# fenghansen/YOND_public

Hardware: AMD Instinct MI355X
Metric: Bayer megapixels/sec end-to-end (NLE+VST+denoise+iVST) (higher is better)
Workload: dtype f32 (3x3 convolutions: f32 operands as two f16 halves -- 22-23 significant bits -- on the f16 MFMA, 3 products per f32 product, f32 accumulate; per-layer error vs float64 asserted <= 2x the f32 direct kernel's and <= 2e-5 of max|ref| (tests/test_hip_conv.py; measured 1.3e-6 vs 1.5e-6), whole frame v

## Files before the change

### include/yond_hip.h

```cpp
#ifndef YOND_HIP_H
#define YOND_HIP_H

#include <stddef.h>
#include <stdint.h>

#ifdef __cplusplus
extern "C" {
#endif

#define YOND_OK 0
#define YOND_EINVAL (-1)
#define YOND_EUNSUPPORTED (-2)

#define YOND_ABI_VERSION 8
int yond_abi_version(void);

int yond_pack_vst_norm_f32(const float* bayer, int H, int W, float* out, int pad_l, int pad_r, int pad_t,
                           int pad_b, int mode, double scale, double gain, double sigma, double lo,
                           double hi, const double* lut_x, const float* lut_y, int lut_n, float* img_max,
                           void* stream);

int yond_pack_vst_norm_biaslut_f32(const float* bayer, int H, int W, float* out, int pad_l, int pad_r, int pad_t,
                                   int pad_b, double scale, double gain, double sigma, double lo, double hi,
                                   const double* lut_x, const double* lut_y, int lut_n, float* img_max, void* stream);
// ... 48 lines not shown
    int kc;
    int algo;
    const float* out4_w;
    const float* out4_b;
    const float* out4_x;
    const float* out4_ub;
    float* out4_dst;
    unsigned int* status;
    int in_fmt, out_fmt;
    int res_fmt;
    unsigned long long* clk;
    int tile_order;
    float* dst2;
} YondConvDesc;
#define YOND_STATUS_HALF_OVERFLOW 1u
#define YOND_FMT_NHWC_F32 0
#define YOND_FMT_SPLIT_PLANES 1
#define YOND_FMT_PLANES4 2
#define YOND_SP_PLANE_UNITS(H, W) ((((H) * (W)) + 8) / 8 * 8)
#define YOND_SP_BYTES(N, C, H, W) ((size_t)(N) * ((C) / 16) * 4 * (size_t)YOND_SP_PLANE_UNITS(H, W) * 16)
#define YOND_HP_BYTES(N, C, H, W) ((size_t)(N) * ((C) / 16) * 2 * (size_t)YOND_SP_PLANE_UNITS(H, W) * 16)

int yond_conv_config(int ksize, int stride, int cin, int cout, int shuffle, int N, int Ho, int Wo, int* tn, int* kc);
int yond_pack_conv_weight_f32(const float* w, int cout, int cin, int ksize, int tn, int kc, float* dst);
int yond_pack_conv_weight_split_f32(const float* w, int cout, int cin, int ksize, int tn, int kc, float* dst);
int yond_conv2d_f32(const YondConvDesc* desc, void* stream);

int yond_conv_wino_supported(int cin, int cout);
int yond_pack_conv_wino_weight_f32(const float* w, int cout, int cin, int tn, float* dst);

int yond_conv_split_supported(int ksize, int stride, int cin, int cout);
int yond_pack_conv_split_weight_f32(const float* w, int cout, int cin, int ksize, int tn, int parts, float* dst);
int yond_gemm_k1_stationary_supported(const YondConvDesc* desc);
int yond_pack_conv_split_weight_dev_f32(const float* w, int cout, int cin, int ksize, int tn, int parts, float* dst, int* status,
                                        void* stream);
int yond_pack_conv_split_weights_batch_dev_f32(const float* src, const long long* desc, int nlayers, float* dst, size_t ngroups,
                                               int* status, void* stream);

int yond_conv_in_f32(const float* x, const float* ub , int N, int H, int W, int Cout,
                     const float* wpk, const float* bias, float slope, float* dst,
                     int out_fmt , void* stream);
int yond_pack_conv_in_weight_f32(const float* w , int cout, float* dst );

int yond_conv_out_f32(const float* feat , int Cin, const float* w ,
                      const float* bias , const float* x ,
                      const float* ub , int N, int H, int W, float* dst ,
                      void* stream);

int yond_maxpool2_f32(const float* src, int N, int H, int W, int C, float* dst, void* stream);

typedef struct YondFilmDesc {
    int kind, C, ld;
    const float *w_a0, *b_a0, *w_a2, *b_a2;
    const float *w_b0, *b_b0;
    const float *w_b, *b_b;
    const float *cb1, *cb2;
    float *s1, *t1, *s2, *t2;
} YondFilmDesc;
int yond_film_f32(const YondFilmDesc* descs, int nblocks, const float* t , const float* ub ,
                  int N, void* stream);

int yond_box_stats_self1_f32(const float* bayer, int H, int W, int k, int k2, int tile_w, float* mean,
                             float* var, float* blur2, void* stream);
int yond_box_stats_self2_f32(const float* blur2, int h, int w, int k, int tile_w, float* lap, void* stream);
int yond_box_stats_collab_f32(const float* bayer_lr, const float* bayer_hr, int H, int W, int k, int tile_w,
                              float* mean, float* var, float* lap, void* stream);
// ... 234 lines not shown
```

### yond_public_amd/_lib.py

```python
import ctypes as C
import os

import torch

_HERE = os.path.dirname(os.path.abspath(__file__))
LIB_PATH = os.environ.get("YOND_HIP_LIB", os.path.join(_HERE, "libyond_hip.so"))
_lib = None
ABI_VERSION = 8

vp, i32, f32, f64, sz, i64 = C.c_void_p, C.c_int, C.c_float, C.c_double, C.c_size_t, C.c_longlong


class YondConvDesc(C.Structure):
    _fields_ = [("src0", vp), ("src1", vp), ("C0", i32), ("C1", i32), ("N", i32), ("H", i32), ("W", i32),
                ("Ho", i32), ("Wo", i32), ("Cout", i32), ("ksize", i32), ("stride", i32), ("shuffle", i32),
                ("pre_act", i32), ("post_act", i32), ("slope", f32), ("wpk", vp), ("escale", vp),
                ("eshift", vp), ("ebatch", i32), ("res", vp), ("dst", vp), ("tn", i32), ("kc", i32), ("algo", i32),
                ("out4_w", vp), ("out4_b", vp), ("out4_x", vp), ("out4_ub", vp), ("out4_dst", vp), ("status", vp),
                ("in_fmt", i32), ("out_fmt", i32), ("res_fmt", i32), ("clk", vp), ("tile_order", i32), ("dst2", vp)]


class YondBlock0Desc(C.Structure):
    _fields_ = [("x", vp), ("in_fmt", i32), ("N", i32), ("H", i32), ("W", i32), ("w1", vp), ("w2", vp),
                ("s1", vp), ("t1", vp), ("s2", vp), ("t2", vp), ("ebatch", i32), ("dst", vp),
# ... 2 lines not shown

class YondFilmDesc(C.Structure):
    _fields_ = [("kind", i32), ("C", i32), ("ld", i32),
                ("w_a0", vp), ("b_a0", vp), ("w_a2", vp), ("b_a2", vp), ("w_b0", vp), ("b_b0", vp),
                ("w_b", vp), ("b_b", vp), ("cb1", vp), ("cb2", vp),
                ("s1", vp), ("t1", vp), ("s2", vp), ("t2", vp)]


PROTOTYPES = {
    "yond_abi_version": [],
    "yond_pack_vst_norm_f32": [vp, i32, i32, vp, i32, i32, i32, i32, i32, f64, f64, f64, f64, f64, vp, vp, i32, vp, vp],
    "yond_pack_vst_norm_biaslut_f32": [vp, i32, i32, vp, i32, i32, i32, i32, f64, f64, f64, f64, f64, vp, vp, i32, vp, vp],
    "yond_bias_eval_f32": [vp, sz, vp, vp, i32, i32, i32, f64, f64, vp, vp],
    "yond_denorm_ivst_unpack_f32": [vp, i32, i32, i32, i32, i32, i32, vp, i32, f64, f64, f64, f64, f64, i32, vp],
    "yond_pack_vst_norm_batch_f32": [vp, i32, i32, i32, vp, i32, i32, i32, i32, f64, f64, f64, f64, f64, vp, vp, i32, i32, vp, vp],
    "yond_denorm_ivst_unpack_batch_f32": [vp, i32, i32, i32, i32, i32, i32, i32, vp, i32, f64, f64, f64, f64, f64, i32, vp],
    "yond_vst_elem_f32": [vp, sz, f64, f64, f64, vp, vp],
    "yond_ivst_elem_f64": [vp, sz, f64, f64, i32, vp, vp],
    "yond_bayer2rggb_f32": [vp, i32, i32, vp, vp],
    "yond_rggb2bayer_f32": [vp, i32, i32, vp, vp],
    "yond_rot90_f32": [vp, i32, i32, i32, i32, vp, vp],
    "yond_nchw4_to_nhwc4_f32": [vp, vp, i32, i32, i32, vp],
    "yond_nhwc4_to_nchw4_f32": [vp, vp, i32, i32, i32, vp],
    "yond_image_max_f32": [vp, i32, sz, vp, vp, vp],
    "yond_conv_config": [i32, i32, i32, i32, i32, i32, i32, i32, C.POINTER(i32), C.POINTER(i32)],
    "yond_pack_conv_weight_f32": [vp, i32, i32, i32, i32, i32, vp],
    "yond_conv2d_f32": [C.POINTER(YondConvDesc), vp],
    "yond_conv_wino_supported": [i32, i32],
    "yond_pack_conv_wino_weight_f32": [vp, i32, i32, i32, vp],
    "yond_pack_conv_weight_split_f32": [vp, i32, i32, i32, i32, i32, vp],
    "yond_conv_split_supported": [i32, i32, i32, i32],
    "yond_pack_conv_split_weight_f32": [vp, i32, i32, i32, i32, i32, vp],
    "yond_gemm_k1_stationary_supported": [C.POINTER(YondConvDesc)],
    "yond_pack_conv_split_weight_dev_f32": [vp, i32, i32, i32, i32, i32, vp, vp, vp],
    "yond_pack_conv_split_weights_batch_dev_f32": [vp, vp, i32, vp, sz, vp, vp],
    "yond_conv_in_f32": [vp, vp, i32, i32, i32, i32, vp, vp, f32, vp, i32, vp],
    "yond_pack_conv_in_weight_f32": [vp, i32, vp],
    "yond_conv_out_f32": [vp, i32, vp, vp, vp, vp, i32, i32, i32, vp, vp],
    "yond_maxpool2_f32": [vp, i32, i32, i32, i32, vp, vp],
    "yond_film_f32": [vp, i32, vp, vp, i32, vp],
    "yond_box_stats_self1_f32": [vp, i32, i32, i32, i32, i32, vp, vp, vp, vp],
    "yond_box_stats_self2_f32": [vp, i32, i32, i32, i32, vp, vp],
    "yond_box_stats_collab_f32": [vp, vp, i32, i32, i32, i32, vp, vp, vp, vp],
    "yond_box_stats_self_stats_f32": [vp, i32, i32, i32, i32, i32, vp, vp, vp, vp, vp, i32, vp, vp],
    "yond_box_stats_collab_stats_f32": [vp, vp, i32, i32, i32, i32, vp, vp, vp, vp, i32, vp, vp],
    "yond_select_ws_bytes": [i32],
    "yond_select_ranks_f32": [vp, sz, vp, i32, vp, vp, vp],
    "yond_percentiles_f32": [vp, sz, vp, i32, vp, vp, vp],
    "yond_nle_ws_bytes": [sz],
    "yond_nle_stats_f32": [vp, vp, sz, i32, vp, i32, vp, vp],
    "yond_nle_threshold_f32": [vp, sz, vp, i32, i32, vp, vp],
    "yond_nle_state_layout": [vp],
    "yond_nle_moments_f32": [vp, vp, vp, sz, vp, vp],
    "yond_nlf_occupancy_f32": [vp, vp, sz, i32, vp, i32, vp, vp],
    "yond_nlf_score3_f64": [vp, vp, vp, i32, vp, vp, vp],
    "yond_nlf_moments_f32": [vp, vp, vp, sz, vp, vp, vp],
    "yond_bias_lut_f64": [vp, i32, f64, f64, vp, vp],
    "yond_block_metrics_tiles": [i32, i32],
    "yond_block_metrics_f32": [vp, vp, i32, i32, i32, i32, vp, vp],
    "yond_block_metrics_rgb8": [vp, vp, i32, i32, i32, i32, vp, vp],
    "yond_render_srgb": [vp, i32, i32, i32, i32, i32, C.POINTER(f64), C.POINTER(f64), i32, vp, vp, i32, vp, f64, vp],
    "yond_clock_probe": [f64, vp, vp],
    "yond_img2raw_f32": [vp, sz, i32, i32, i32, vp, vp, i32, i32, i32, vp, vp, vp, vp],
    "yond_pg_noise_f32": [vp, vp, sz, i32, vp, i32, vp],
    "yond_camera_noise_f32": [vp, vp, sz, i32, vp, i32, i32, vp],
    "yond_est_conv_in_f32": [vp, i32, i32, i32, i32, vp, vp, vp, vp],
# ... 133 lines not shown
```

### yond_public_amd/csrc/conv.hip

```cpp
#include "common.h"
#include <cstdlib>

#ifndef YOND_B32_WGS
#define YOND_B32_WGS 2
#endif
#ifndef YOND_ABL
#define YOND_ABL 0
#endif

template <int KS, int STRIDE, int TH, int TN, int KC>
struct ConvCfg {
    static constexpr int TW = 32;
    static constexpr int TAPS = KS * KS;
    static constexpr int PADK = KS / 2;
    static constexpr int IH = (TH - 1) * STRIDE + KS;
    static constexpr int IW = (TW - 1) * STRIDE + KS;
    static constexpr int HALF = (IW + 1) / 2;
    static constexpr int TWP = (STRIDE == 2) ? 2 * HALF : IW;
    static constexpr int PS = KC + 4;
    static constexpr int IN_FLOATS = IH * TWP * PS;
    static constexpr int Q = KC / 8;
    static constexpr int W_FLOATS = TAPS * Q * 2 * TN * 4;
    static constexpr int BUF_FLOATS = IN_FLOATS + W_FLOATS;
    static constexpr int NW = TN / 32;
// ... 487 lines not shown
            for (int tap = 0; tap < taps; ++tap)
                for (int q = 0; q < Q; ++q)
                    for (int h = 0; h < 2; ++h)
                        for (int j = 0; j < tn; ++j)
                            for (int e = 0; e < 4; ++e) {
                                const int co = ct * tn + j, ci = ch * kc + q * 8 + h * 4 + e;
                                dst[o++] = w[((size_t)co * cin + ci) * taps + tap];
                            }
    return YOND_OK;
}

extern "C" int yond_pack_conv_weight_split_f32(const float* w, int cout, int cin, int ksize, int tn, int kc, float* dst) {
    const int rc = yond_pack_conv_weight_f32(w, cout, cin, ksize, tn, kc, dst);
    if (rc != YOND_OK) return rc;
    const size_t n = (size_t)cout * cin * ksize * ksize;
    for (size_t i = 0; i < n; ++i)
        if (!(fabsf(w[i]) <= 65504.0f)) return YOND_EUNSUPPORTED;
    for (size_t i = 0; i < n; ++i) {
        const float v = dst[i];
        const _Float16 h = (_Float16)v;
        const _Float16 l = (_Float16)((v - (float)h) * 2048.0f);
        unsigned short hb, lb;
        __builtin_memcpy(&hb, &h, 2);
        __builtin_memcpy(&lb, &l, 2);
        const unsigned u = (unsigned)hb | ((unsigned)lb << 16);
        __builtin_memcpy(&dst[i], &u, 4);
    }
    return YOND_OK;
}

int yond_conv_wino_dispatch(const YondConvDesc& d, hipStream_t st);
int yond_conv_split_dispatch(const YondConvDesc& d, hipStream_t st);
int yond_gemm_k1_stationary_dispatch(const YondConvDesc& d, hipStream_t st);

extern "C" int yond_conv2d_f32(const YondConvDesc* dp, void* stream) {
    if (!dp) return YOND_EINVAL;
    const YondConvDesc& d = *dp;
    hipStream_t st = (hipStream_t)stream;
    if (!d.src0 || !(d.dst || d.out4_dst) || !d.wpk || d.N <= 0 || d.H <= 0 || d.W <= 0 || d.Ho <= 0 || d.Wo <= 0) return YOND_EINVAL;
    if (d.out4_dst && ((d.algo != 3 && d.algo != 4) || !d.out4_w || d.Cout != 32 || d.stride != 1)) return YOND_EUNSUPPORTED;
    if (d.C1 > 0 && !d.src1) return YOND_EINVAL;
    if (d.shuffle < 0 || d.shuffle > 2) return YOND_EINVAL;
    if (d.shuffle == 2 && d.algo != 3 && d.algo != 4 && d.algo != 6) return YOND_EUNSUPPORTED;
    if ((long long)d.N * d.H * d.W > 0x7fffffffLL) return YOND_EUNSUPPORTED;
    if (d.pre_act != 0 && d.pre_act != 1) return YOND_EINVAL;
    if (d.in_fmt < 0 || d.in_fmt > 2 || d.out_fmt < 0 || d.out_fmt > 2 || (d.res_fmt != 0 && d.res_fmt != 2)) return YOND_EINVAL;
    if (d.algo == 6) return yond_gemm_k1_stationary_dispatch(d, st);
    if ((d.in_fmt || d.out_fmt || d.res_fmt) && d.algo != 3 && d.algo != 4) return YOND_EUNSUPPORTED;
    if (d.algo == 1) return yond_conv_wino_dispatch(d, st);
    if (d.algo == 3 || d.algo == 4) return yond_conv_split_dispatch(d, st);
    if (d.algo != 0 && d.algo != 2 && d.algo != 5) return YOND_EINVAL;
    if (d.tn != 32 && d.tn != 64) return YOND_EINVAL;
    int tn, kc;
    const int rc = yond_conv_config(d.ksize, d.stride, d.C0 + d.C1, d.Cout, d.shuffle, 0, 0, 0, &tn, &kc);
    if (rc != YOND_OK) return rc;
    tn = d.tn;
    if (d.kc != 0) kc = d.kc;
    if (kc != 8 && kc != 16) return YOND_EINVAL;
    if (kc == 8 && d.ksize != 3) return YOND_EINVAL;
    if (d.ksize == 3 && d.stride == 2 && kc != 8) return YOND_EINVAL;
    if (d.C0 % kc != 0 || d.C1 % kc != 0 || d.Cout % tn != 0) return YOND_EUNSUPPORTED;
    if (d.shuffle && (d.ksize != 1 || (d.Cout / 4) % tn != 0)) return YOND_EUNSUPPORTED;
    if ((long long)d.N * d.H * d.W > 0x7fffffffLL) return YOND_EUNSUPPORTED;
    if (d.stride == 2) {
        if (d.Ho != (d.H + 1) / 2 || d.Wo != (d.W + 1) / 2) return YOND_EINVAL;
    } else if (d.Ho != d.H || d.Wo != d.W) return YOND_EINVAL;
    if (d.pre_act != 0 && d.pre_act != 1) return YOND_EINVAL;
    if (d.post_act != 0 && d.post_act != 2) return YOND_EUNSUPPORTED;
    if (d.pre_act == 1 && !(d.ksize == 3 && d.stride == 1)) return YOND_EUNSUPPORTED;
    if (d.ksize == 3 && d.stride == 1 && kc == 8) {
        if (d.pre_act) return tn == 64 ? launch_conv<3, 1, 8, 64, 8, true>(d, st) : launch_conv<3, 1, 8, 32, 8, true>(d, st);
        return tn == 64 ? launch_conv<3, 1, 8, 64, 8, false>(d, st) : launch_conv<3, 1, 8, 32, 8, false>(d, st);
    }
    if (d.ksize == 3 && d.stride == 1) {
        if (d.pre_act) return tn == 64 ? launch_conv<3, 1, 8, 64, 16, true>(d, st) : launch_conv<3, 1, 8, 32, 16, true>(d, st);
        return tn == 64 ? launch_conv<3, 1, 8, 64, 16, false>(d, st) : launch_conv<3, 1, 8, 32, 16, false>(d, st);
    }
    if (d.ksize == 3 && d.stride == 2)
        return tn == 64 ? launch_conv<3, 2, 8, 64, 8, false>(d, st) : launch_conv<3, 2, 4, 32, 8, false>(d, st);
    return tn == 64 ? launch_conv<1, 1, 8, 64, 16, false>(d, st) : launch_conv<1, 1, 8, 32, 16, false>(d, st);
// ... 2 lines not shown
```

### yond_public_amd/engine.py

```python
import ctypes as C
import os

import numpy as np
import torch

from . import _lib as L


def _rup(c, m=32):
    return (c + m - 1) // m * m


def _np_ptr(a):
    return C.c_void_p(a.ctypes.data)


FILM_MAX_C = 1024


WINO_DEFAULT = 'split'


SPLIT_PLANES = True
SP_FLOW = True
HALF_FLOW = True
HALF_K1_TN128 = True
HALF_S2_TN128 = True
HALF_FLOW_TN128 = True
HALF_TN128 = True
FUSE_OUT4 = True
FUSE_BLOCK0 = False
K1_SUB2 = True
K1_D2_LEVELS = (3,)
K1_STATIONARY_LEVELS = (2, 1, 0)
K1_D2_LEVELS_HALF = ()
SP_CONV1_MIN_LEVEL = 3
UNET_SP = True
SNAKE_ORDER = True


def sp_plane_units(H, W):
    return (H * W + 8) // 8 * 8


class _PackedConv:

    def __init__(self, dev, weight, bias, ksize, stride, splits, shuffle=False):
        lib = L.load()
        w = weight.detach().to('cpu', torch.float32).numpy()
        if shuffle:
            cin, cout = w.shape[0], w.shape[1]
            coutp = _rup(cout)
            m = np.zeros((4, coutp, cin), np.float32)
            m[:, :cout, :] = w.transpose(2, 3, 1, 0).reshape(4, cout, cin)
            w = m.reshape(4 * coutp, cin, 1, 1)
            self.cout_real_p = coutp
            gemm_n = 4 * coutp
        else:
            cout = w.shape[0]
            coutp = _rup(cout)
            gemm_n = coutp
            self.cout_real_p = coutp
        assert sum(splits) == w.shape[1], (splits, w.shape)
        psplits = [_rup(s) for s in splits]
        cinp = sum(psplits)
        wp = np.zeros((gemm_n, cinp, ksize, ksize), np.float32)
        so, do = 0, 0
# ... 214 lines not shown
            return False
        prec = getattr(self, 'precision', 'fp32')
        if prec not in ('fp32', 'fp16'):
            return False
        parts = 2 if prec == 'fp32' else 1
        return all(pc.ksize == 3 and pc.stride == 1 and pc.split(parts) is not None for pc in (pc1, pc2))

    def _sp_flow(self, N, H, W):
        if not (SPLIT_PLANES and SP_FLOW) or getattr(self, 'strict', False) or getattr(self, 'conv_algo', WINO_DEFAULT) != 'split':
            return False
        prec = getattr(self, 'precision', 'fp32')
        if prec not in ('fp32', 'fp16') or (prec == 'fp16' and not HALF_FLOW) or sp_plane_units(H, W) * 64 * 4 >= 2 ** 31:
            return False
        parts = 2 if prec == 'fp32' else 1
        for i, blk in self.blocks.items():
            for k in ('conv1', 'conv2', 'pool', 'upsc'):
                if k in blk and blk[k].split(parts, wide=False) is None:
                    return False
        return self._out4_fusable(self.blocks[9]['conv2'], flow=True)

    def _out4_fusable(self, pc, flow=False):
        prec = getattr(self, 'precision', 'fp32')
        return (not getattr(self, 'strict', False) and getattr(self, 'conv_algo', WINO_DEFAULT) == 'split' and (prec == 'fp32' or (prec == 'fp16' and flow))
                and pc.ksize == 3 and pc.stride == 1 and pc.gemm_n == 32 and pc.split(2 if prec == 'fp32' else 1) is not None and FUSE_OUT4)

    def _new_sp(self, key, N, H, W, Cc, parts=2):
        cache = self.__dict__.setdefault('_sp_cache', {})
        k = (key, N, H, W, Cc, parts, getattr(self, 'lane', 0))
        if k not in cache:
            cache[k] = torch.zeros(N * (Cc // 16) * 2 * parts * sp_plane_units(H, W) * 4, dtype=torch.float32, device=self.dev)
        return cache[k]

    def _conv(self, pc, src0, src1, N, H, W, dst, escale=None, eshift=None, ebatch=0, res=None, pre_act=0, post_act=0,
              slope=0.0, algo=None, out4=None, in_fmt=0, out_fmt=0, res_fmt=0, dst2=None, stationary=False):
        d = L.YondConvDesc()
        d.src0 = src0.data_ptr()
        d.src1 = src1.data_ptr() if src1 is not None else None
        d.C0 = pc.psplits[0]
        d.C1 = pc.psplits[1] if len(pc.psplits) > 1 else 0
        d.N, d.H, d.W = N, H, W
        if pc.stride == 2:
            d.Ho, d.Wo = (H + 1) // 2, (W + 1) // 2
        else:
            d.Ho, d.Wo = H, W
        d.Cout = pc.gemm_n
        d.ksize, d.stride, d.shuffle = pc.ksize, pc.stride, int(pc.shuffle)
        d.pre_act, d.post_act, d.slope = pre_act, post_act, slope
        prec = getattr(self, 'precision', 'fp32')
        if getattr(self, 'strict', False) and algo is None:
            prec, algo = 'fp32-mfma', 1
        if algo is None:
            algo = getattr(self, 'conv_algo', WINO_DEFAULT)
            if prec == 'fp32-mfma' and algo == 'split':
                algo = 1
            if prec == 'fp16' and WINO_DEFAULT == 'split':
                algo = 'half'
        fp16 = prec == 'fp16' or algo == 'fp16'
        wino = split = None
        if algo in ('split', 'half'):
            ws2 = (HALF_S2_TN128 and algo == 'half' and pc.stride == 2 and in_fmt == 1 and out_fmt == 2 and dst2 is None
                   and (pc.gemm_n // 128) * ((d.Wo + 31) // 32) * ((d.Ho + 7) // 8) * N >= 256)
            ws2 = ws2 or (HALF_K1_TN128 and algo == 'half' and pc.ksize == 1 and in_fmt == 1 and dst2 is None)
            split = pc.split(2 if algo == 'split' else 1, wide=(not (in_fmt or out_fmt or res_fmt or dst2 is not None)) or (HALF_FLOW_TN128 and out_fmt == 1),
                             wide_s2=ws2)
            if algo == 'half' and pc.ksize == 1 and in_fmt != 1:
                split = None
            if split is None and not fp16 and pc.ksize == 3:
                wino = pc.wino()
        elif not fp16:
            wino = pc.wino() if algo in (1, 2) else None
        if split is not None:
            tn, wpk = split
            kc = 16
            d.algo = 3 if algo == 'split' else 4
        elif wino is not None:
            tn, wpk = wino
            kc = 8
            d.algo = 1
        elif algo == 'split' and pc.ksize == 1 and not fp16 and pc.config(N, d.Ho, d.Wo, split=True)[2] is not None:
            tn, kc, wpk = pc.config(N, d.Ho, d.Wo, split=True)
            d.algo = 5
        else:
            tn, kc, wpk = pc.config(N, d.Ho, d.Wo)
            d.algo = 2 if (fp16 and pc.wmax <= 65504.0) else 0
        d.wpk = wpk.data_ptr()
        d.tn = tn
        d.kc = kc
        d.escale = escale.data_ptr() if escale is not None else None
        d.eshift = (eshift if eshift is not None else pc.bias).data_ptr()
        d.ebatch = ebatch
        d.res = res.data_ptr() if res is not None else None
        d.dst = dst.data_ptr() if dst is not None else None
        status = getattr(self, 'status', None)
        d.status = status.data_ptr() + 4 * self.status_slot if status is not None else None
        d.in_fmt, d.out_fmt, d.res_fmt = in_fmt, out_fmt, res_fmt
        d.dst2 = dst2.data_ptr() if dst2 is not None else None
        if stationary and d.algo == 3 and self.lib.yond_gemm_k1_stationary_supported(C.byref(d)):
            d.algo = 6
        if SNAKE_ORDER and d.algo in (3, 4, 6):
            self._tile_order = 1 - getattr(self, '_tile_order', 0)
            d.tile_order = self._tile_order
        clk = getattr(self, 'clk', None)
        d.clk = clk.data_ptr() if (clk is not None and d.algo in (3, 4, 6)) else None
        if (in_fmt or out_fmt or res_fmt) and d.algo not in (3, 4, 6):
            raise L.YondHipError("split-plane / 4-channel-plane tensors need the split-operand kernel (algo 3, or 4 with h-only planes)")
        if out4 is not None:
            w4, b4, x4, ub4, o4 = out4
            if d.algo not in (3, 4):
                raise L.YondHipError("fused output projection needs the split-operand 3x3 kernel")
            d.out4_w, d.out4_b = w4.data_ptr(), (b4.data_ptr() if b4 is not None else None)
            d.out4_x = x4.data_ptr() if x4 is not None else None
            d.out4_ub = ub4.data_ptr() if ub4 is not None else None
            d.out4_dst = o4.data_ptr()
        prof = getattr(self, 'prof', None)
        if prof is not None:
            tag = f"conv_wino_kernel<{tn}>" if d.algo == 1 else f"conv_mfma_kernel<{pc.ksize},{pc.stride},8,{tn},{kc}>"
            if d.algo in (3, 4, 6):
                tag = f"conv_split_kernel<{pc.stride if pc.ksize == 3 else 'k1'},{tn},{1 if d.algo == 4 else 2}>" + ("/stationary" if d.algo == 6 else "")
            if d.algo == 2:
                tag += "/f16"
            if d.algo == 5:
                tag += "/split"
            only = getattr(self, 'prof_only', None)
            if only is not None and not only(tag):
                prof = None
            every = getattr(self, 'prof_every', 1)
            if every > 1 and getattr(self, '_fwd_idx', 0) % every:
                prof = None
        if prof is not None:
            e0, e1 = torch.cuda.Event(enable_timing=True), torch.cuda.Event(enable_timing=True)
            e0.record()
        L.check(self.lib.yond_conv2d_f32(C.byref(d), L.stream()), "yond_conv2d_f32")
        if prof is not None:
            e1.record()
            prof.append((tag, 2.0 * pc.macs_per_pixel * N * d.Ho * d.Wo, e0, e1))
        return dst

    def _block0_weights(self, pc):
        w = getattr(pc, '_b0', None)
        if w is None:
            if not L.has("yond_pack_block0_weight_f32"):
                raise L.YondHipError("the fused level-0 block exists only in experiment builds of the library (python -m yond_public_amd.build --experiments)")
            if not (pc.ksize == 3 and pc.stride == 1 and pc.gemm_n == 32 and pc.cinp == 32 and len(pc.psplits) == 1):
                return None
            host = np.zeros(9 * 2 * 4 * 32 * 8, np.float16)
            if self.lib.yond_pack_block0_weight_f32(_np_ptr(pc._wp), 32, 32, _np_ptr(host)) != 0:
                return None
            w = pc._b0 = torch.from_numpy(host.view(np.float32)).to(pc._dev)
        return w

    def _block0(self, pc1, pc2, x, N, H, W, f, in_fmt, dst=None, out4=None):
# ... 107 lines not shown
            L.check(lib.yond_conv_in_f32(L.ptr(x4), L.ptr(ub), N, H, W, nfp, L.ptr(self.conv_in_w), L.ptr(self.conv_in_b),
                                         0.01, L.ptr(a), P4 if flow else 0, st), "yond_conv_in_f32")
            skips = {}
            h, w = H, W
            cur = a
            xsp = None
            for i in range(1, 10):
                blk = self.blocks[i]
                cp = blk['Cp']
                f = film[f'conv{i}']
                last = i == 9
                xfmt = P4 if (flow and not last) else 0
                if i >= 6:
                    xs = self._new(N, 2 * h, 2 * w, cp)
                    up = blk['upsc2'] if (flow and K1_SUB2 and 'upsc2' in blk) else blk['upsc']
                    xsp = (self._new_sp(('xspd', i), N, 2 * h, 2 * w, cp, pt)
                           if (flow and not last and (9 - i) in (K1_D2_LEVELS if pt == 2 else K1_D2_LEVELS_HALF) and up is blk['upsc'] and cp % 64 == 0 and w > 16) else None)
                    self._conv(up, cur, skips[10 - i], N, h, w, xs, in_fmt=SP if flow else 0, out_fmt=xfmt, dst2=xsp,
                               stationary=(9 - i) in K1_STATIONARY_LEVELS)
                    h, w = 2 * h, 2 * w
                    cur = xs
                if flow and FUSE_BLOCK0 and h == H and cp == 32 and self._block0_weights(blk['conv1']) is not None and self._block0_weights(blk['conv2']) is not None:
                    if last and self._out4_fusable(blk['conv2'], flow):
                        out4 = self._new(N, H, W, 4)
                        self._block0(blk['conv1'], blk['conv2'], cur, N, h, w, f, xfmt, out4=(self.w_out, self.b_out, x4 if self.res else None, ub, out4))
                        return out4
                    if not last:
                        out = self._new_sp(('out', i), N, h, w, cp, pt)
                        self._block0(blk['conv1'], blk['conv2'], cur, N, h, w, f, xfmt, dst=out)
                        cur = out
                        skips[i] = cur
                        nxt = self._new(N, h // 2, w // 2, blk['pool'].coutp)
                        xsp = self._new_sp(('xsp', i + 1), N, h // 2, w // 2, blk['pool'].coutp, pt) if (flow and i >= SP_CONV1_MIN_LEVEL) else None
                        self._conv(blk['pool'], cur, None, N, h, w, nxt, in_fmt=SP, out_fmt=P4, dst2=xsp)
                        h, w = h // 2, w // 2
                        cur = nxt
                        continue
                act_in_producer = self._split_pair(blk['conv1'], blk['conv2'])
                sp = SP if (flow or (act_in_producer and SPLIT_PLANES and getattr(self, 'precision', 'fp32') == 'fp32'
                                      and sp_plane_units(h, w) * 64 < 2 ** 31)) else 0
                tmp = self._new_sp(('tmp', i), N, h, w, cp, pt) if sp else self._new(N, h, w, cp)
                if xsp is not None and sp and act_in_producer:
                    self._conv(blk['conv1'], xsp, None, N, h, w, tmp, escale=f[0], eshift=f[1], ebatch=1, pre_act=0, post_act=1,
                               in_fmt=SP, out_fmt=sp)
                else:
                    self._conv(blk['conv1'], cur, None, N, h, w, tmp, escale=f[0], eshift=f[1], ebatch=1, pre_act=1,
                               post_act=1 if act_in_producer else 0, in_fmt=xfmt, out_fmt=sp)
                xsp = None
                pre2 = 0 if act_in_producer else 1
                if last and self._out4_fusable(blk['conv2'], flow):
                    out4 = self._new(N, H, W, 4)
                    self._conv(blk['conv2'], tmp, None, N, h, w, None, escale=f[2], eshift=f[3], ebatch=1, res=cur, pre_act=pre2,
                               out4=(self.w_out, self.b_out, x4 if self.res else None, ub, out4), in_fmt=sp)
                    return out4
                if flow:
                    out = self._new_sp(('out', i), N, h, w, cp, pt)
                    self._conv(blk['conv2'], tmp, None, N, h, w, out, escale=f[2], eshift=f[3], ebatch=1, res=cur, pre_act=pre2,
                               in_fmt=SP, out_fmt=SP, res_fmt=P4)
                else:
                    out = self._new(N, h, w, cp)
                    self._conv(blk['conv2'], tmp, None, N, h, w, out, escale=f[2], eshift=f[3], ebatch=1, res=cur, pre_act=pre2, in_fmt=sp)
                cur = out
                if i <= 4:
                    skips[i] = cur
                    nxt = self._new(N, h // 2, w // 2, blk['pool'].coutp)
                    xsp = self._new_sp(('xsp', i + 1), N, h // 2, w // 2, blk['pool'].coutp, pt) if (flow and i >= SP_CONV1_MIN_LEVEL) else None
                    self._conv(blk['pool'], cur, None, N, h, w, nxt, in_fmt=SP if flow else 0, out_fmt=P4 if flow else 0, dst2=xsp)
                    h, w = h // 2, w // 2
                    cur = nxt
            feat = cur
        else:
            a = self._new(N, H, W, nfp)
            L.check(lib.yond_conv_in_f32(L.ptr(x4), L.ptr(ub), N, H, W, nfp, L.ptr(self.conv_in_w), L.ptr(self.conv_in_b),
                                         0.2, L.ptr(a), 0, st), "yond_conv_in_f32")
            cv = self.convs
            h, w = H, W
            cur = self._conv(cv['conv1_2'], a, None, N, h, w, self._new(N, h, w, cv['conv1_2'].coutp), post_act=2, slope=0.2)
            skips = {1: cur}

            def first_of_pair(i, c1, c2, s0, s1):
                sp = (UNET_SP and SPLIT_PLANES and not getattr(self, 'strict', False) and getattr(self, 'conv_algo', WINO_DEFAULT) == 'split'
                      and getattr(self, 'precision', 'fp32') == 'fp32' and c1.split(2) is not None and c2.split(2) is not None
                      and N * sp_plane_units(h, w) * 64 < 2 ** 31)
                dst = self._new_sp(('utmp', i), N, h, w, c1.coutp) if sp else self._new(N, h, w, c1.coutp)
                self._conv(c1, s0, s1, N, h, w, dst, post_act=2, slope=0.2, out_fmt=1 if sp else 0)
                return dst, (1 if sp else 0)

            for i in range(2, 6):
                cpv = cur.shape[-1]
                pooled = self._new(N, h // 2, w // 2, cpv)
                L.check(lib.yond_maxpool2_f32(L.ptr(cur), N, h, w, cpv, L.ptr(pooled), st), "yond_maxpool2_f32")
                h, w = h // 2, w // 2
                c1, c2 = cv[f'conv{i}_1'], cv[f'conv{i}_2']
                cur, fmt = first_of_pair(i, c1, c2, pooled, None)
                cur = self._conv(c2, cur, None, N, h, w, self._new(N, h, w, c2.coutp), post_act=2, slope=0.2, in_fmt=fmt)
                if i < 5:
                    skips[i] = cur
            for i in range(6, 10):
                upc = cv[f'upv{i}']
                up = self._new(N, 2 * h, 2 * w, upc.cout_real_p)
# ... 48 lines not shown
```

Baseline: 2700.

## Add tall-tile stride-2 split-plane conv kernel for downsampling levels

Adds a dedicated persistent kernel for 3x3 stride-2 downsampling convolutions that read split-plane f16 input and write 4-channel planes. It uses an 8-row by 32-column output tile with 64 output channels, double-buffered weight DMA into LDS, and prefetch of the next input chunk interleaved with the MFMA schedule. The engine routes the pool convolutions of levels 0-2 to this kernel when it is supported, falling back otherwise. The aim is better input reuse and overlap than the generic split kernel gives on large stride-2 layers, at the cost of a large LDS footprint and another code path to maintain.

```diff
diff --git a/include/yond_hip.h b/include/yond_hip.h
--- a/include/yond_hip.h
+++ b/include/yond_hip.h
@@ -104,6 +104,7 @@
 int yond_conv_split_supported(int ksize, int stride, int cin, int cout);
 int yond_pack_conv_split_weight_f32(const float* w, int cout, int cin, int ksize, int tn, int parts, float* dst);
 int yond_gemm_k1_stationary_supported(const YondConvDesc* desc);
+int yond_conv_s2_tall_supported(const YondConvDesc* desc);
 int yond_pack_conv_split_weight_dev_f32(const float* w, int cout, int cin, int ksize, int tn, int parts, float* dst, int* status,
                                         void* stream);
 int yond_pack_conv_split_weights_batch_dev_f32(const float* src, const long long* desc, int nlayers, float* dst, size_t ngroups,
diff --git a/yond_public_amd/_lib.py b/yond_public_amd/_lib.py
--- a/yond_public_amd/_lib.py
+++ b/yond_public_amd/_lib.py
@@ -58,6 +58,7 @@
     "yond_conv_split_supported": [i32, i32, i32, i32],
     "yond_pack_conv_split_weight_f32": [vp, i32, i32, i32, i32, i32, vp],
     "yond_gemm_k1_stationary_supported": [C.POINTER(YondConvDesc)],
+    "yond_conv_s2_tall_supported": [C.POINTER(YondConvDesc)],
     "yond_pack_conv_split_weight_dev_f32": [vp, i32, i32, i32, i32, i32, vp, vp, vp],
     "yond_pack_conv_split_weights_batch_dev_f32": [vp, vp, i32, vp, sz, vp, vp],
     "yond_conv_in_f32": [vp, vp, i32, i32, i32, i32, vp, vp, f32, vp, i32, vp],
diff --git a/yond_public_amd/csrc/conv.hip b/yond_public_amd/csrc/conv.hip
--- a/yond_public_amd/csrc/conv.hip
+++ b/yond_public_amd/csrc/conv.hip
@@ -543,6 +543,7 @@
 int yond_conv_wino_dispatch(const YondConvDesc& d, hipStream_t st);
 int yond_conv_split_dispatch(const YondConvDesc& d, hipStream_t st);
 int yond_gemm_k1_stationary_dispatch(const YondConvDesc& d, hipStream_t st);
+int yond_conv_s2_tall_dispatch(const YondConvDesc& d, hipStream_t st);
 
 extern "C" int yond_conv2d_f32(const YondConvDesc* dp, void* stream) {
     if (!dp) return YOND_EINVAL;
@@ -557,6 +558,7 @@
     if (d.pre_act != 0 && d.pre_act != 1) return YOND_EINVAL;
     if (d.in_fmt < 0 || d.in_fmt > 2 || d.out_fmt < 0 || d.out_fmt > 2 || (d.res_fmt != 0 && d.res_fmt != 2)) return YOND_EINVAL;
     if (d.algo == 6) return yond_gemm_k1_stationary_dispatch(d, st);
+    if (d.algo == 7) return yond_conv_s2_tall_dispatch(d, st);
     if ((d.in_fmt || d.out_fmt || d.res_fmt) && d.algo != 3 && d.algo != 4) return YOND_EUNSUPPORTED;
     if (d.algo == 1) return yond_conv_wino_dispatch(d, st);
     if (d.algo == 3 || d.algo == 4) return yond_conv_split_dispatch(d, st);
diff --git a/yond_public_amd/csrc/conv_s2_tall.hip b/yond_public_amd/csrc/conv_s2_tall.hip
--- /dev/null
+++ b/yond_public_amd/csrc/conv_s2_tall.hip
@@ -0,0 +1,357 @@
+#include "common.h"
+
+typedef _Float16 f16x8 __attribute__((ext_vector_type(8)));
+typedef _Float16 f16x4 __attribute__((ext_vector_type(4)));
+#define S2T_GLOBAL __attribute__((address_space(1)))
+
+namespace {
+constexpr int S2T_TH = 8;
+constexpr int S2T_IH = (S2T_TH - 1) * 2 + 3;
+constexpr int S2T_IW = 31 * 2 + 3;
+constexpr int S2T_HALF = (S2T_IW + 1) / 2;
+constexpr int S2T_TWP = 2 * S2T_HALF;
+constexpr int S2T_PLANE = S2T_IH * S2T_TWP * 4;
+constexpr int S2T_IMG = 4 * S2T_PLANE + 4;
+constexpr int S2T_W = 9 * 2 * 2 * 64 * 4;
+constexpr int S2T_NWV = S2T_W / 4;
+constexpr int S2T_NWT = (S2T_NWV + 511) / 512;
+constexpr int S2T_NITEM = S2T_IH * S2T_IW * 4;
+constexpr int S2T_NIN = (S2T_NITEM + 511) / 512;
+constexpr int S2T_FILM = 1536;
+constexpr int S2T_W_OFF = S2T_IMG, S2T_FILM_OFF = S2T_W_OFF + 2 * S2T_W;
+constexpr int S2T_SMEM = (S2T_FILM_OFF + 2 * S2T_FILM) * 4;
+static_assert(S2T_SMEM <= 160 * 1024, "LDS budget");
+static_assert((S2T_NIN - 1) * 512 < S2T_NITEM, "only a thread's last item may lie past the tile");
+
+__device__ __forceinline__ float s2t_silu(float x) {
+    return x * __builtin_amdgcn_rcpf(1.0f + __builtin_amdgcn_exp2f(x * -1.44269504088896341f));
+}
+}
+
+template <bool D2>
+__global__ __launch_bounds__(512) void conv_s2_tall_kernel(const YondConvDesc d) {
+    extern __shared__ __attribute__((aligned(16))) float smem[];
+    const int tid = threadIdx.x, lane = tid & 63, wave = __builtin_amdgcn_readfirstlane(tid >> 6);
+    const int li = lane & 31, lh = lane >> 5;
+    const int rg = wave & 3, cg = wave >> 2;
+    const int nct = d.Cout / 64, ntx = (d.Wo + 31) / 32, nty = (d.Ho + S2T_TH - 1) / S2T_TH;
+    const int total = nct * ntx * nty * d.N;
+    const int G = gridDim.x;
+    const int lslot = (G % 8 == 0) ? (blockIdx.x % 8) * (G / 8) + blockIdx.x / 8 : blockIdx.x;
+    const int nchunk = d.C0 / 16;
+    const bool rev = d.tile_order != 0;
+    const int PS0 = YOND_SP_PLANE_UNITS(d.H, d.W);
+    if (lslot >= total) return;
+    const bool clk_on = d.clk != nullptr && blockIdx.x == 0 && tid == 0;
+    unsigned long long clk_c0 = 0, clk_r0 = 0;
+    if (clk_on) { clk_c0 = __builtin_amdgcn_s_memtime(); clk_r0 = __builtin_amdgcn_s_memrealtime(); }
+    asm volatile("" : "+v"(clk_c0), "+v"(clk_r0));
+    float* dst_v = d.dst;
+    char* dst2_v = (char*)d.dst2;
+    unsigned int* word_v = d.status;
+    unsigned long long* clk_v = d.clk;
+    asm volatile("" : "+v"(dst_v), "+v"(dst2_v), "+v"(word_v), "+v"(clk_v));
+    int nct_v = nct, ntx_v = ntx, nty_v = nty;
+    unsigned ps2_v = (unsigned)YOND_SP_PLANE_UNITS(d.Ho, d.Wo);
+    asm volatile("" : "+v"(nct_v), "+v"(ntx_v), "+v"(nty_v), "+v"(ps2_v));
+
+    {
+        const int nf = (d.ebatch ? d.N : 1) * d.Cout;
+        for (int i = tid; i < nf; i += 512) {
+            smem[S2T_FILM_OFF + i] = d.escale ? d.escale[i] : 1.0f;
+            smem[S2T_FILM_OFF + S2T_FILM + i] = d.eshift ? d.eshift[i] : 0.0f;
+        }
+    }
+
+    int in_lds[S2T_NIN];
+#pragma unroll
+    for (int k = 0; k < S2T_NIN; ++k) {
+        const int it = tid + k * 512;
+        const int pix = it >> 2, py = pix / S2T_IW, px = pix % S2T_IW;
+        const int lp = py * S2T_TWP + (px & 1) * S2T_HALF + (px >> 1);
+        in_lds[k] = it < S2T_NITEM ? (it & 3) * S2T_PLANE + lp * 4 : 4 * S2T_PLANE;
+    }
+
+    struct Tile { int ct, n, ox0, oy0; };
+    auto origin = [&](int t) {
+        Tile T;
+        int b = t;
+        T.ct = b % nct_v; b /= nct_v;
+        const int tx = b % ntx_v; b /= ntx_v;
+        const int ty = b % nty_v, n = b / nty_v;
+        T.n = __builtin_amdgcn_readfirstlane(rev ? d.N - 1 - n : n);
+        T.ct = __builtin_amdgcn_readfirstlane(T.ct);
+        T.ox0 = __builtin_amdgcn_readfirstlane((rev ? ntx_v - 1 - tx : tx) * 32);
+        T.oy0 = __builtin_amdgcn_readfirstlane((rev ? nty_v - 1 - ty : ty) * S2T_TH);
+        return T;
+    };
+    unsigned voff[S2T_NIN];
+    auto decode = [&](const Tile& T) {
+#pragma unroll
+        for (int k = 0; k < S2T_NIN; ++k) {
+            const int it = tid + k * 512;
+            const int pix = it >> 2, py = pix / S2T_IW, px = pix % S2T_IW;
+            const int gy = T.oy0 * 2 - 1 + py, gx = T.ox0 * 2 - 1 + px;
+            const bool in = it < S2T_NITEM && gy >= 0 && gy < d.H && gx >= 0 && gx < d.W;
+            voff[k] = ((unsigned)(it & 3) * (unsigned)PS0 + (unsigned)(in ? gy * d.W + gx : d.H * d.W)) * 16u;
+        }
+    };
+    auto uniform_ptr = [&](const void* p) {
+        const unsigned long long a = (unsigned long long)(uintptr_t)p;
+        const unsigned lo = __builtin_amdgcn_readfirstlane((unsigned)a), hi = __builtin_amdgcn_readfirstlane((unsigned)(a >> 32));
+        return (const char*)(uintptr_t)(((unsigned long long)hi << 32) | lo);
+    };
+    auto in_base = [&](const Tile& T, int ch) { return (const char*)d.src0 + (size_t)(T.n * nchunk + ch) * 4 * (size_t)PS0 * 16; };
+    auto w_base = [&](const Tile& T, int ch) { return uniform_ptr(d.wpk + ((size_t)T.ct * nchunk + ch) * S2T_W); };
+    f32x4 vin[S2T_NIN];
+    auto issue_load = [&](auto kc, const char* ib) __attribute__((always_inline)) {
+        constexpr int k = decltype(kc)::value;
+        vin[k] = *(const S2T_GLOBAL f32x4*)(const S2T_GLOBAL char*)(ib + voff[k]);
+    };
+    auto issue_dma = [&](auto kc, const char* wsrc, float* wbuf) __attribute__((always_inline)) {
+        constexpr int k = decltype(kc)::value;
+        const unsigned lds0 = (unsigned)(uintptr_t)(__attribute__((address_space(3))) float*)wbuf;
+        const int it = tid + k * 512;
+        const int it_wave = __builtin_amdgcn_readfirstlane(it - lane);
+        const unsigned lds_wave = __builtin_amdgcn_readfirstlane(lds0 + (unsigned)it_wave * 16u);
+        const unsigned vo = (unsigned)it * 16u;
+        if ((k + 1) * 512 <= S2T_NWV || it_wave < S2T_NWV)
+            asm volatile("s_mov_b32 m0, %0\n\ts_nop 0\n\tglobal_load_lds_dwordx4 %1, %2" ::"s"(lds_wave), "v"(vo), "s"(wsrc) : "memory");
+    };
+    auto write_in = [&]() __attribute__((always_inline)) {
+#pragma unroll
+        for (int k = 0; k < S2T_NIN; ++k) *(f32x4*)(smem + in_lds[k]) = vin[k];
+    };
+
+    f32x16 acc[2][2];
+    auto zero_acc = [&]() {
+#pragma unroll
+        for (int a = 0; a < 2; ++a)
+#pragma unroll
+            for (int m = 0; m < 2; ++m)
+#pragma unroll
+                for (int r = 0; r < 16; ++r) acc[a][m][r] = 0.0f;
+    };
+
+    const int x_off = (lh * 2) * S2T_PLANE + ((rg * 4) * S2T_TWP + li) * 4;
+    const int w_off = ((lh * 2) * 64 + cg * 32 + li) * 4;
+    const bool wave_hi = wave >= 4;
+    const char* ib_s = nullptr;
+    const char* wsrc_s = nullptr;
+    auto mfma_step = [&](const float* wcur, float* wnext, auto&& prep) __attribute__((always_inline)) {
+        typedef const __attribute__((address_space(3))) f16x8* lds_h8;
+        const __attribute__((address_space(3))) float* xb = (const __attribute__((address_space(3))) float*)(smem + x_off);
+        const __attribute__((address_space(3))) float* wb = (const __attribute__((address_space(3))) float*)(wcur + w_off);
+        constexpr int R = 5, NQ = 3 * R, XD = 3, Q0 = 2, NQW = NQ - Q0, NOPS = S2T_NWT + S2T_NIN;
+        f16x8 xr[XD][2], wt[2][3][2];
+        auto loadX = [&](auto qc) __attribute__((always_inline)) {
+            constexpr int q = decltype(qc)::value, dx = q / R, r = q % R;
+            constexpr int xo = (dx & 1) * S2T_HALF + (dx >> 1);
+#pragma unroll
+            for (int p = 0; p < 2; ++p) xr[q % XD][p] = *(lds_h8)(xb + p * S2T_PLANE + (r * S2T_TWP + xo) * 4);
+        };
+        auto loadW = [&](auto dc) __attribute__((always_inline)) {
+            constexpr int dx = decltype(dc)::value;
+#pragma unroll
+            for (int dy = 0; dy < 3; ++dy)
+#pragma unroll
+                for (int p = 0; p < 2; ++p) wt[dx % 2][dy][p] = *(lds_h8)(wb + (((dy * 3 + dx) * 4 + p) * 64) * 4);
+        };
+        loadW(IntC<0>{});
+        loadX(IntC<0>{});
+        loadX(IntC<1>{});
+        static_for<0, NQ>([&](auto qc) __attribute__((always_inline)) {
+            constexpr int q = decltype(qc)::value, dx = q / R, r = q % R;
+            constexpr bool wpre = r == 2 && dx < 2;
+            if constexpr (q + 2 < NQ) loadX(IntC<q + 2>{});
+            if constexpr (wpre) loadW(IntC<dx + 1>{});
+            constexpr int nmf = 3 * ((r <= 2 ? 1 : 0) + (r >= 2 ? 1 : 0));
+#pragma unroll
+            for (int a = 0; a < 3; ++a) {
+#pragma unroll
+                for (int m = 0; m < 2; ++m) {
+                    const int dy = r - 2 * m;
+                    if (dy < 0 || dy > 2) continue;
+                    acc[a == 1 ? 0 : 1][m] = __builtin_amdgcn_mfma_f32_32x32x16_f16(wt[dx % 2][dy][a == 2 ? 1 : 0], xr[q % XD][a == 0 ? 1 : 0],
+                                                                                    acc[a == 1 ? 0 : 1][m], 0, 0, 0);
+                }
+            }
+            if constexpr (q == 0) { if (wave_hi) __builtin_amdgcn_s_setprio(1); }
+            if constexpr (q == NQ / 2) { if (wave_hi) __builtin_amdgcn_s_setprio(0); }
+            if constexpr (q == Q0 - 1) prep();
+            constexpr int qq = q >= Q0 ? q - Q0 : 0;
+            constexpr int o_lo = q >= Q0 ? (qq * NOPS + NQW - 1) / NQW : 0, o_hi = q >= Q0 ? ((qq + 1) * NOPS + NQW - 1) / NQW : 0;
+            static_for<o_lo, (o_hi < NOPS ? o_hi : NOPS)>([&](auto oc) __attribute__((always_inline)) {
+                constexpr int o = decltype(oc)::value;
+                if constexpr (o < S2T_NWT) issue_dma(IntC<o>{}, wsrc_s, wnext);
+                else issue_load(IntC<o - S2T_NWT>{}, ib_s);
+            });
+            constexpr int nrd = (q + 2 < NQ ? 2 : 0) + (wpre ? 6 : 0);
+            constexpr int l_lo = o_lo > S2T_NWT ? o_lo : S2T_NWT, nld = o_hi > l_lo ? o_hi - l_lo : 0;
+            if constexpr (nrd > 0) __builtin_amdgcn_sched_group_barrier(0x100, nrd, 0);
+#pragma unroll
+            for (int i = 0; i < nmf; ++i) {
+                __builtin_amdgcn_sched_group_barrier(0x008, 1, 0);
+                if (i == 0 && nld > 0) __builtin_amdgcn_sched_group_barrier(0x020, nld, 0);
+            }
+        });
+    };
+
+    float slope_eff = d.post_act == 2 ? d.slope : 1.0f;
+    asm volatile("" : "+v"(slope_eff));
+    YondRange amax;
+    auto epilogue = [&](const Tile& T) __attribute__((always_inline)) {
+        const int ox = T.ox0 + li;
+        const bool col_ok = ox < d.Wo;
+        const int cbase = T.ct * 64 + cg * 32 + 4 * lh;
+        const float* fs = smem + S2T_FILM_OFF + (d.ebatch ? T.n * d.Cout : 0) + cbase;
+        const long long hw = (long long)d.Ho * d.Wo;
+        f32x4 es[4], et[4];
+#pragma unroll
+        for (int g = 0; g < 4; ++g) {
+            es[g] = *(const f32x4*)(fs + 8 * g);
+            et[g] = *(const f32x4*)(fs + S2T_FILM + 8 * g);
+        }
+#pragma unroll
+        for (int m = 0; m < 2; ++m) {
+            const int oy = T.oy0 + rg * 2 + m;
+            const bool ok = col_ok && oy < d.Ho;
+            const long long pixo = (long long)oy * d.Wo + ox;
+            float* op = dst_v + (((long long)T.n * (d.Cout / 4) + cbase / 4) * hw + pixo) * 4;
+            const long long gstep = 8LL * hw;
+#pragma unroll
+            for (int g = 0; g < 4; ++g) {
+                f32x4 v;
+#pragma unroll
+                for (int e = 0; e < 4; ++e) {
+                    float x = acc[0][m][4 * g + e];
+                    x = fmaf(acc[1][m][4 * g + e], 1.0f / 2048.0f, x);
+                    x = fmaf(x, es[g][e], et[g][e]);
+                    x = x > 0.0f ? x : x * slope_eff;
+                    v[e] = x + 0.0f;
+                }
+                if (ok) *(S2T_GLOBAL f32x4*)(S2T_GLOBAL float*)(op + g * gstep) = v;
+                if constexpr (D2) {
+                    f32x4 a;
+#pragma unroll
+                    for (int e = 0; e < 4; ++e) a[e] = s2t_silu(v[e]);
+                    amax.add(a);
+                    const f16x4 h = {(_Float16)a[0], (_Float16)a[1], (_Float16)a[2], (_Float16)a[3]};
+                    const int c8 = cbase - 4 * lh + 8 * g;
+                    const size_t PS2 = (size_t)ps2_v;
+                    char* pp = dst2_v + ((size_t)(((T.n * (d.Cout / 16) + (c8 >> 4)) * 2 + ((c8 >> 3) & 1)) * 2) * PS2 + (size_t)pixo) * 16 + lh * 8;
+                    if (ok) *(S2T_GLOBAL f16x4*)(S2T_GLOBAL char*)pp = h;
+                    const f16x4 l = {(_Float16)((a[0] - (float)h[0]) * 2048.0f), (_Float16)((a[1] - (float)h[1]) * 2048.0f),
+                                     (_Float16)((a[2] - (float)h[2]) * 2048.0f), (_Float16)((a[3] - (float)h[3]) * 2048.0f)};
+                    if (ok) *(S2T_GLOBAL f16x4*)(S2T_GLOBAL char*)(pp + PS2 * 16) = l;
+                }
+            }
+        }
+    };
+
+    struct Cur { int tile, ch; };
+    auto adv = [&](Cur c) {
+        Cur n;
+        const bool last = c.ch + 1 == nchunk;
+        n.tile = last ? c.tile + G : c.tile;
+        n.ch = last ? 0 : c.ch + 1;
+        return n;
+    };
+    Cur cs = {lslot, 0};
+    Tile lt = origin(lslot), cur = lt;
+    auto park = [&](Tile& T) { asm volatile("" : "+v"(T.ct), "+v"(T.n), "+v"(T.ox0), "+v"(T.oy0)); };
+    park(cur);
+    float* w0 = smem + S2T_W_OFF;
+    float* w1 = w0 + S2T_W;
+    decode(lt);
+    {
+        const char* ws = w_base(lt, 0);
+        const char* ib = in_base(lt, 0);
+        static_for<0, S2T_NWT>([&](auto kc) __attribute__((always_inline)) { issue_dma(kc, ws, w0); });
+        static_for<0, S2T_NIN>([&](auto kc) __attribute__((always_inline)) { issue_load(kc, ib); });
+    }
+    zero_acc();
+    asm volatile("s_waitcnt vmcnt(0)" ::: "memory");
+    write_in();
+    asm volatile("s_waitcnt vmcnt(0) lgkmcnt(0)\n\ts_barrier" ::: "memory");
+    while (true) {
+        const bool last_ch = cs.ch + 1 == nchunk;
+        const Cur cn = adv(cs);
+        auto prep = [&]() __attribute__((always_inline)) {
+            if (last_ch && cn.tile < total) {
+                lt = origin(cn.tile);
+                decode(lt);
+            }
+            ib_s = in_base(lt, cn.ch);
+            wsrc_s = w_base(lt, cn.ch);
+        };
+        mfma_step(w0, w1, prep);
+        asm volatile("s_waitcnt lgkmcnt(0)\n\ts_barrier" ::: "memory");
+        asm volatile("s_waitcnt vmcnt(0)" ::: "memory");
+        write_in();
+        if (last_ch) {
+            epilogue(cur);
+            zero_acc();
+            cur = lt;
+            park(cur);
+        }
+        asm volatile("s_waitcnt lgkmcnt(0)\n\ts_barrier" ::: "memory");
+        if (cn.tile >= total) break;
+        cs = cn;
+        float* t = w0;
+        w0 = w1;
+        w1 = t;
+    }
+    if constexpr (D2) {
+        if (word_v && !amax.at_most(65504.0f)) atomicOr(word_v, YOND_STATUS_HALF_OVERFLOW);
+    }
+    if (clk_on) {
+        atomicAdd(clk_v, __builtin_amdgcn_s_memtime() - clk_c0);
+        atomicAdd(clk_v + 1, __builtin_amdgcn_s_memrealtime() - clk_r0);
+    }
+}
+
+static bool s2t_takes(const YondConvDesc& d) {
+    if (d.ksize != 3 || d.stride != 2 || d.shuffle != 0 || d.tn != 64 || !d.src0 || d.src1 || d.C1 != 0 || !d.dst || !d.wpk) return false;
+    if (d.in_fmt != YOND_FMT_SPLIT_PLANES || d.out_fmt != YOND_FMT_PLANES4 || d.res_fmt || d.res || d.out4_dst || d.pre_act) return false;
+    if (d.post_act != 0 && d.post_act != 2) return false;
+    if (d.N <= 0 || d.H <= 0 || d.W <= 0 || d.Ho != (d.H + 1) / 2 || d.Wo != (d.W + 1) / 2) return false;
+    if (d.C0 <= 0 || d.C0 % 16 || d.Cout <= 0 || d.Cout % 64) return false;
+    if ((long long)(d.ebatch ? d.N : 1) * d.Cout > S2T_FILM) return false;
+    if ((long long)d.N * d.H * d.W > 0x7fffffffLL) return false;
+    if ((long long)d.N * (d.C0 / 16) * 4 * YOND_SP_PLANE_UNITS(d.H, d.W) * 4 >= 0x7fffffffLL) return false;
+    if ((long long)YOND_SP_PLANE_UNITS(d.H, d.W) * 16 * 4 >= 0x7fffffffLL) return false;
+    const long long tiles = (long long)(d.Cout / 64) * ((d.Wo + 31) / 32) * ((d.Ho + S2T_TH - 1) / S2T_TH) * d.N;
+    if (tiles > 0x7fffffffLL) return false;
+    if (d.Wo <= 16) {
+        const int f = d.Wo <= 8 ? 4 : 2;
+        const long long subs = (long long)d.N * ((d.Ho + 3) / 4) * ((d.Wo + 32 / f - 1) / (32 / f));
+        const long long tiles_f = (long long)(d.Cout / 64) * ((subs + f - 1) / f), tiles4 = (long long)(d.Cout / 64) * ((d.Ho + 3) / 4) * d.N;
+        const bool fits = (long long)d.H * d.W * d.C0 * 4 * f < (1LL << 31);
+        if (fits && (tiles_f + 255) / 256 < (tiles4 + 255) / 256) return false;
+    }
+    return true;
+}
+
+extern "C" int yond_conv_s2_tall_supported(const YondConvDesc* d) { return (d && (d->algo == 3 || d->algo == 7) && s2t_takes(*d)) ? 1 : 0; }
+
+template <bool D2>
+static int launch_s2t(const YondConvDesc& d, hipStream_t st) {
+    static bool attr_set = false;
+    auto kern = conv_s2_tall_kernel<D2>;
+    if (!attr_set) {
+        hipError_t e = hipFuncSetAttribute((const void*)kern, hipFuncAttributeMaxDynamicSharedMemorySize, S2T_SMEM);
+        if (e != hipSuccess) return (int)e;
+        attr_set = true;
+    }
+    const long long total = (long long)(d.Cout / 64) * ((d.Wo + 31) / 32) * ((d.Ho + S2T_TH - 1) / S2T_TH) * d.N;
+    const int grid = total < 256 ? (int)total : 256;
+    hipLaunchKernelGGL(kern, dim3(grid), dim3(512), S2T_SMEM, st, d);
+    YOND_LAUNCH_CHECK();
+    return YOND_OK;
+}
+
+int yond_conv_s2_tall_dispatch(const YondConvDesc& d, hipStream_t st) {
+    if (!s2t_takes(d)) return YOND_EUNSUPPORTED;
+    return d.dst2 ? launch_s2t<true>(d, st) : launch_s2t<false>(d, st);
+}
diff --git a/yond_public_amd/engine.py b/yond_public_amd/engine.py
--- a/yond_public_amd/engine.py
+++ b/yond_public_amd/engine.py
@@ -33,6 +33,7 @@
 K1_SUB2 = True
 K1_D2_LEVELS = (3,)
 K1_STATIONARY_LEVELS = (2, 1, 0)
+S2_TALL_LEVELS = (0, 1, 2)
 K1_D2_LEVELS_HALF = ()
 SP_CONV1_MIN_LEVEL = 3
 UNET_SP = True
@@ -313,7 +314,7 @@
         return cache[k]
 
     def _conv(self, pc, src0, src1, N, H, W, dst, escale=None, eshift=None, ebatch=0, res=None, pre_act=0, post_act=0,
-              slope=0.0, algo=None, out4=None, in_fmt=0, out_fmt=0, res_fmt=0, dst2=None, stationary=False):
+              slope=0.0, algo=None, out4=None, in_fmt=0, out_fmt=0, res_fmt=0, dst2=None, stationary=False, s2_tall=False):
         d = L.YondConvDesc()
         d.src0 = src0.data_ptr()
         d.src1 = src1.data_ptr() if src1 is not None else None
@@ -378,12 +379,14 @@
         d.dst2 = dst2.data_ptr() if dst2 is not None else None
         if stationary and d.algo == 3 and self.lib.yond_gemm_k1_stationary_supported(C.byref(d)):
             d.algo = 6
-        if SNAKE_ORDER and d.algo in (3, 4, 6):
+        if s2_tall and d.algo == 3 and pc.ksize == 3 and pc.stride == 2 and self.lib.yond_conv_s2_tall_supported(C.byref(d)):
+            d.algo = 7
+        if SNAKE_ORDER and d.algo in (3, 4, 6, 7):
             self._tile_order = 1 - getattr(self, '_tile_order', 0)
             d.tile_order = self._tile_order
         clk = getattr(self, 'clk', None)
-        d.clk = clk.data_ptr() if (clk is not None and d.algo in (3, 4, 6)) else None
-        if (in_fmt or out_fmt or res_fmt) and d.algo not in (3, 4, 6):
+        d.clk = clk.data_ptr() if (clk is not None and d.algo in (3, 4, 6, 7)) else None
+        if (in_fmt or out_fmt or res_fmt) and d.algo not in (3, 4, 6, 7):
             raise L.YondHipError("split-plane / 4-channel-plane tensors need the split-operand kernel (algo 3, or 4 with h-only planes)")
         if out4 is not None:
             w4, b4, x4, ub4, o4 = out4
@@ -396,8 +399,8 @@
         prof = getattr(self, 'prof', None)
         if prof is not None:
             tag = f"conv_wino_kernel<{tn}>" if d.algo == 1 else f"conv_mfma_kernel<{pc.ksize},{pc.stride},8,{tn},{kc}>"
-            if d.algo in (3, 4, 6):
-                tag = f"conv_split_kernel<{pc.stride if pc.ksize == 3 else 'k1'},{tn},{1 if d.algo == 4 else 2}>" + ("/stationary" if d.algo == 6 else "")
+            if d.algo in (3, 4, 6, 7):
+                tag = f"conv_split_kernel<{pc.stride if pc.ksize == 3 else 'k1'},{tn},{1 if d.algo == 4 else 2}>" + ("/stationary" if d.algo == 6 else "/tall" if d.algo == 7 else "")
             if d.algo == 2:
                 tag += "/f16"
             if d.algo == 5:
@@ -571,7 +574,7 @@
                         skips[i] = cur
                         nxt = self._new(N, h // 2, w // 2, blk['pool'].coutp)
                         xsp = self._new_sp(('xsp', i + 1), N, h // 2, w // 2, blk['pool'].coutp, pt) if (flow and i >= SP_CONV1_MIN_LEVEL) else None
-                        self._conv(blk['pool'], cur, None, N, h, w, nxt, in_fmt=SP, out_fmt=P4, dst2=xsp)
+                        self._conv(blk['pool'], cur, None, N, h, w, nxt, in_fmt=SP, out_fmt=P4, dst2=xsp, s2_tall=(i - 1) in S2_TALL_LEVELS)
                         h, w = h // 2, w // 2
                         cur = nxt
                         continue
@@ -604,7 +607,7 @@
                     skips[i] = cur
                     nxt = self._new(N, h // 2, w // 2, blk['pool'].coutp)
                     xsp = self._new_sp(('xsp', i + 1), N, h // 2, w // 2, blk['pool'].coutp, pt) if (flow and i >= SP_CONV1_MIN_LEVEL) else None
-                    self._conv(blk['pool'], cur, None, N, h, w, nxt, in_fmt=SP if flow else 0, out_fmt=P4 if flow else 0, dst2=xsp)
+                    self._conv(blk['pool'], cur, None, N, h, w, nxt, in_fmt=SP if flow else 0, out_fmt=P4 if flow else 0, dst2=xsp, s2_tall=(i - 1) in S2_TALL_LEVELS)
                     h, w = h // 2, w // 2
                     cur = nxt
             feat = cur
```

After: 2733, median of 6. 1.2% higher.
